# sylvainma/Summarizer

Measured on AMD Instinct MI355X. Metric: frames scored/sec (T x 1024), higher is better.
Workload: dtype f32; 1 GPU; vasnet score, S-TVSum: 50 videos/GPU, T~U(150,320) (sum 12003), D=1024, packed batch; parallelism=video-sharded x1

## Files before the change

summarizer_amd/csrc/attn_b16.hip:

```cpp
#include "pw_common.h"
#include <math.h>
#include <cstdlib>
#include <algorithm>
#include <vector>

namespace sumk {

namespace {

constexpr int AT_ROWS = 64, AT_TMAX = 320, AT_BK = 64;
constexpr int AT_PP = 2 * AT_TMAX + 16;
constexpr int AT_NCH = 256;
constexpr int AT_ROWB = 2 * AT_BK;
constexpr int AT_CROW = 2 * AT_NCH;
constexpr int AT_NST = 3;
constexpr int AT_STAGE1 = (AT_TMAX + AT_ROWS) * AT_ROWB;
constexpr int AT_STAGE2 = AT_BK * AT_CROW;
constexpr int AT_SP = 0;
constexpr int AT_ST2 = 43008;
constexpr int AT_RED = 3 * AT_STAGE1;
constexpr int AT_LDS = AT_RED + 8 * 64 * 4;
static_assert(AT_ROWS * AT_PP <= AT_ST2 && AT_ST2 + 3 * AT_STAGE2 <= AT_RED && AT_LDS <= 160 * 1024, "LDS map");

typedef unsigned int u32x4 __attribute__((ext_vector_type(4)));
typedef float f32x4v __attribute__((ext_vector_type(4)));
typedef __bf16 bf16x4v __attribute__((ext_vector_type(4)));

__device__ __forceinline__ u32x2 pack_bf16x4(float a, float b, float c, float d) {
  return __builtin_bit_cast(u32x2, __builtin_convertvector(f32x4v{a, b, c, d}, bf16x4v));
}


template <bool BWD, int NJ>
__device__ __forceinline__ void attn_strip_body(const AttnStripArgs& a, const SeqInfo& si, const int strip, char* const lds) {
  const int tid = threadIdx.x, lane = tid & 63, li = lane & 31, lh = lane >> 5;
  const int wave = __builtin_amdgcn_readfirstlane(tid >> 6);
  const int T = si.T, i0 = strip * AT_ROWS;
  const Drop drop = drop_resolve(a.drop);
  constexpr int T64 = NJ * 64;
  constexpr int NTW = (2 * NJ + 3) / 4;
  const int D = a.D;
  const int rows = min(AT_ROWS, T - i0);

  const __amdgpu_buffer_rsrc_t rA = __builtin_amdgcn_make_buffer_rsrc(
      const_cast<unsigned short*>(a.A16 + (int64_t)(si.row0 + i0) * a.lda), (short)0, ((rows - 1) * a.lda + D) * 2, 0x00020000);
  const __amdgpu_buffer_rsrc_t rB = __builtin_amdgcn_make_buffer_rsrc(
      const_cast<unsigned short*>(a.B16 + (int64_t)si.row0 * a.ldb), (short)0, ((T - 1) * a.ldb + D) * 2, 0x00020000);
  const int d_row = wave * 8 + (lane >> 3);
  const int d_chunk = (lane & 7) ^ (((lane >> 4) + 4 * (wave & 1)) & 7);
  int vk[NJ];
#pragma unroll
  for (int p = 0; p < NJ; ++p) vk[p] = (min(d_row + 64 * p, T - 1) * a.ldb + d_chunk * 8) * 2;
  const int vq = (min(d_row, rows - 1) * a.lda + d_chunk * 8) * 2;
  constexpr int NI1 = NJ + 1;
  auto dma1 = [&](int kt, int stage) {
    char* const dst = lds + stage * AT_STAGE1 + wave * 1024;
#pragma unroll
    for (int p = 0; p < NJ; ++p)
      __builtin_amdgcn_raw_ptr_buffer_load_lds(rB, (lds_vptr)(dst + p * 8192), 16, vk[p], kt * (AT_BK * 2), 0, 0);
    __builtin_amdgcn_raw_ptr_buffer_load_lds(rA, (lds_vptr)(dst + T64 * AT_ROWB), 16, vq, kt * (AT_BK * 2), 0, 0);
  };
  const int qt = wave & 1, kg = wave >> 1;
  const int sw = (li >> 1) & 7;
  const int fq = (T64 + qt * 32 + li) * AT_ROWB, fk = (kg * 32 + li) * AT_ROWB;
  struct Frag1 { bf16x8 bq, ak[NTW]; };
  auto read1 = [&](const char* buf, int ks, Frag1& f) {
    const int so = ((2 * ks + lh) ^ sw) * 16;
    f.bq = *reinterpret_cast<const bf16x8*>(buf + fq + so);
#pragma unroll
    for (int j = 0; j < NTW; ++j) f.ak[j] = *reinterpret_cast<const bf16x8*>(buf + fk + j * 128 * AT_ROWB + so);
  };
  f32x16 acc[NTW];
#pragma unroll
  for (int j = 0; j < NTW; ++j)
#pragma unroll
    for (int r = 0; r < 16; ++r) acc[j][r] = 0.f;

  const int qi = qt * 32 + li, i = i0 + qi;
  const uint64_t drow = (uint64_t)(si.row0 + i) << 20;
  uint32_t keepm[NTW];
#pragma unroll
  for (int j = 0; j < NTW; ++j) keepm[j] = 0u;
  auto keep_step = [&](int r) {
#pragma unroll
    for (int j = 0; j < NTW; ++j) {
      const int key = (kg + 4 * j) * 32 + 8 * (r >> 2) + 4 * lh + (r & 3);
      keepm[j] |= (dropout_keep(drop.seed, 0, drow | (uint64_t)key, drop.thr) ? 1u : 0u) << r;
    }
  };
  const int KT1 = D / AT_BK;
  dma1(0, 0);
  if (AT_NST > 2) dma1(1, 1);
  int stage = 0;
  for (int kt = 0; kt < KT1; ++kt) {
    if (AT_NST > 2 && kt + 1 < KT1) wait_vm<NI1>(); else wait_vm<0>();
    __builtin_amdgcn_s_barrier();
    const int st2 = stage == 0 ? AT_NST - 1 : stage - 1;
    const char* const cur = lds + stage * AT_STAGE1;
    auto compute1 = [&]() {
      if (drop.thr && kt < 16) keep_step(kt);
      Frag1 f[2];
      read1(cur, 0, f[0]);
#pragma unroll
      for (int ks = 0; ks < AT_BK / 16; ++ks) {
        if (ks + 1 < AT_BK / 16) read1(cur, ks + 1, f[(ks + 1) & 1]);
#pragma unroll
        for (int j = 0; j < NTW; ++j) acc[j] = __builtin_amdgcn_mfma_f32_32x32x16_bf16(f[ks & 1].ak[j], f[ks & 1].bq, acc[j], 0, 0, 0);
      }
    };
    if (wave < 4) {
      if (kt + AT_NST - 1 < KT1) dma1(kt + AT_NST - 1, st2);
      compute1();
    } else {
      compute1();
      if (kt + AT_NST - 1 < KT1) dma1(kt + AT_NST - 1, st2);
    }
    stage = stage == AT_NST - 1 ? 0 : stage + 1;
  }
  if (drop.thr)
    for (int r = KT1; r < 16; ++r) keep_step(r);
  __syncthreads();

  const __amdgpu_buffer_rsrc_t rC = __builtin_amdgcn_make_buffer_rsrc(
      const_cast<unsigned short*>(a.C16 + (int64_t)si.row0 * a.ldc), (short)0, ((T - 1) * a.ldc + D) * 2, 0x00020000);
  const int c_row = wave * 2 + (lane >> 5);
  const int c_chunk = ((((lane & 31) >> 2) ^ (c_row & 3)) << 2) | (lane & 3);
  const int NC = D / AT_NCH, n_it = NC * NJ;
  constexpr int NI2 = 4;
  auto dma2 = [&](int nc, int kt, int stage) {
    char* const dst = lds + AT_ST2 + stage * AT_STAGE2 + wave * 1024;
#pragma unroll
    for (int p = 0; p < 4; ++p)
      __builtin_amdgcn_raw_ptr_buffer_load_lds(rC, (lds_vptr)(dst + p * 8192), 16,
                                               (min(kt * 64 + c_row + 16 * p, T - 1) * a.ldc + nc * AT_NCH + c_chunk * 8) * 2, 0, 0, 0);
  };
  dma2(0, 0, 0);
  if (n_it > 1) dma2(NJ > 1 ? 0 : 1, NJ > 1 ? 1 : 0, 1);

  const bool row_ok = i < T;
  float* const red = reinterpret_cast<float*>(lds + AT_RED);
  float* const erow = a.E + si.eoff + (int64_t)i * si.ldE;
  unsigned short* const prow = a.P16 + si.e16off + (int64_t)i * T64;
  char* const lrow = lds + AT_SP + qi * AT_PP;
  if constexpr (!BWD) {
    float m = -INFINITY;
#pragma unroll
    for (int j = 0; j < NTW; ++j)
#pragma unroll
      for (int r = 0; r < 16; ++r) {
        const int key = (kg + 4 * j) * 32 + 8 * (r >> 2) + 4 * lh + (r & 3);
        const float e = key < T ? masked_logit(acc[j][r], a.scale, i, key, a.ignore_self, a.aperture) : -INFINITY;
        acc[j][r] = e;
        m = fmaxf(m, e);
      }
    m = fmaxf(m, __shfl_xor(m, 32));
    if (lh == 0) red[kg * 64 + qi] = m;
    lds_barrier();
    m = fmaxf(fmaxf(red[qi], red[64 + qi]), fmaxf(red[128 + qi], red[192 + qi]));
    float sum = 0.f;
#pragma unroll
    for (int j = 0; j < NTW; ++j)
#pragma unroll
      for (int r = 0; r < 16; ++r) {
        const int key = (kg + 4 * j) * 32 + 8 * (r >> 2) + 4 * lh + (r & 3);
        const float p = key < T ? __expf(acc[j][r] - m) : 0.f;
        acc[j][r] = p;
        sum += p;
      }
    sum += __shfl_xor(sum, 32);
    if (lh == 0) red[256 + kg * 64 + qi] = sum;
    lds_barrier();
    sum = (red[256 + qi] + red[320 + qi]) + (red[384 + qi] + red[448 + qi]);
    const float rsum = 1.0f / sum;
#pragma unroll
    for (int j = 0; j < NTW; ++j)
#pragma unroll
      for (int g = 0; g < 4; ++g) {
        const int k0 = (kg + 4 * j) * 32 + 8 * g + 4 * lh;
        if (k0 >= T64) continue;
        float al[4], ad[4];
#pragma unroll
        for (int c = 0; c < 4; ++c) {
          al[c] = k0 + c < T ? acc[j][4 * g + c] * rsum : 0.f;
          ad[c] = drop.thr ? (((keepm[j] >> (4 * g + c)) & 1u) ? al[c] * drop.scale : 0.f) : al[c];
        }
        const u32x2 pk = pack_bf16x4(ad[0], ad[1], ad[2], ad[3]);
        if (row_ok) {
          if (k0 < si.ldE) *reinterpret_cast<float4*>(erow + k0) = make_float4(al[0], al[1], al[2], al[3]);
          *reinterpret_cast<u32x2*>(prow + k0) = pk;
        }
        *reinterpret_cast<u32x2*>(lrow + k0 * 2) = row_ok ? pk : u32x2{0u, 0u};
      }
  } else {
    float dot = 0.f;
    float al[NTW][16];
#pragma unroll
    for (int j = 0; j < NTW; ++j)
#pragma unroll
      for (int g = 0; g < 4; ++g) {
        const int k0 = (kg + 4 * j) * 32 + 8 * g + 4 * lh;
        float4 t = make_float4(0.f, 0.f, 0.f, 0.f);
        if (row_ok && k0 < si.ldE) t = *reinterpret_cast<const float4*>(erow + k0);
        al[j][4 * g] = t.x; al[j][4 * g + 1] = t.y; al[j][4 * g + 2] = t.z; al[j][4 * g + 3] = t.w;
      }
#pragma unroll
    for (int j = 0; j < NTW; ++j)
#pragma unroll
      for (int r = 0; r < 16; ++r) {
        float d = acc[j][r];
        if (drop.thr) d = ((keepm[j] >> r) & 1u) ? d * drop.scale : 0.f;
        acc[j][r] = d;
        dot += d * al[j][r];
      }
    dot += __shfl_xor(dot, 32);
    if (lh == 0) red[kg * 64 + qi] = dot;
    lds_barrier();
    dot = (red[qi] + red[64 + qi]) + (red[128 + qi] + red[192 + qi]);
#pragma unroll
    for (int j = 0; j < NTW; ++j)
#pragma unroll
      for (int g = 0; g < 4; ++g) {
        const int k0 = (kg + 4 * j) * 32 + 8 * g + 4 * lh;
        if (k0 >= T64) continue;
        float v[4];
#pragma unroll
        for (int c = 0; c < 4; ++c) v[c] = al[j][4 * g + c] * (acc[j][4 * g + c] - dot) * a.scale;
        const u32x2 pk = row_ok ? pack_bf16x4(v[0], v[1], v[2], v[3]) : u32x2{0u, 0u};
        if (row_ok) *reinterpret_cast<u32x2*>(prow + k0) = pk;
        *reinterpret_cast<u32x2*>(lrow + k0 * 2) = pk;
      }
  }

  const int rr = (lane >> 2) & 3;
  const int fct = (8 * lh + ((lane & 15) >> 2)) * AT_CROW + 32 * ((lane >> 4) & 1) + 8 * (lane & 3) + ((wave ^ rr) << 6);
  const char* const fp = lds + AT_SP + li * AT_PP + 16 * lh;
  struct Frag2 { bf16x8 fa, fb[2]; };
  auto read2 = [&](const char* buf, int kt, int ks, Frag2& f) {
    f.fa = tr_frag(buf + fct + 16 * ks * AT_CROW, AT_CROW);
#pragma unroll
    for (int u = 0; u < 2; ++u) f.fb[u] = *reinterpret_cast<const bf16x8*>(fp + u * 32 * AT_PP + (kt * 64 + ks * 16) * 2);
  };
  int stage2 = 0, it = 0;
  int nc2 = NJ > 2 ? 0 : (NJ == 2 ? 1 : 2), kt2 = NJ > 2 ? 2 : 0;
  for (int nc = 0; nc < NC; ++nc) {
    f32x16 o[2];
#pragma unroll
    for (int u = 0; u < 2; ++u)
#pragma unroll
      for (int r = 0; r < 16; ++r) o[u][r] = 0.f;
#pragma unroll
    for (int kt = 0; kt < NJ; ++kt) {
      if (it + 1 < n_it && !(kt == 0 && nc > 0)) wait_vm<NI2>(); else wait_vm<0>();
      __builtin_amdgcn_s_waitcnt(0xC07F);
      __builtin_amdgcn_s_barrier();
      const int st2 = stage2 == 0 ? 2 : stage2 - 1;
      const char* const cur = lds + AT_ST2 + stage2 * AT_STAGE2;
      auto compute2 = [&]() {
        Frag2 f[2];
        read2(cur, kt, 0, f[0]);
#pragma unroll
        for (int ks = 0; ks < 4; ++ks) {
          if (ks + 1 < 4) read2(cur, kt, ks + 1, f[(ks + 1) & 1]);
#pragma unroll
          for (int u = 0; u < 2; ++u) o[u] = __builtin_amdgcn_mfma_f32_32x32x16_bf16(f[ks & 1].fa, f[ks & 1].fb[u], o[u], 0, 0, 0);
        }
      };
      if (wave < 4) {
        if (it + 2 < n_it) dma2(nc2, kt2, st2);
        compute2();
      } else {
        compute2();
        if (it + 2 < n_it) dma2(nc2, kt2, st2);
      }
      if (++kt2 == NJ) { kt2 = 0; ++nc2; }
      stage2 = stage2 == 2 ? 0 : stage2 + 1;
      ++it;
    }
#pragma unroll
    for (int u = 0; u < 2; ++u) {
      const int q = u * 32 + li;
      unsigned short* const orow = a.O16 + (int64_t)(si.row0 + i0 + q) * a.ldo + nc * AT_NCH + wave * 32 + 4 * lh;
      if (q < rows) {
#pragma unroll
        for (int g = 0; g < 4; ++g)
          *reinterpret_cast<u32x2*>(orow + 8 * g) = pack_bf16x4(o[u][4 * g], o[u][4 * g + 1], o[u][4 * g + 2], o[u][4 * g + 3]);
      }
    }
  }
}

template <bool BWD>
__global__ __launch_bounds__(512) void attn_strip_kernel(AttnStripArgs a) {
  extern __shared__ __attribute__((aligned(16))) char lds[];
  int s, strip;
  SeqInfo si;
  if (!locate_block(a.seq, a.n_seq, [](int t) { return (t + AT_ROWS - 1) / AT_ROWS; }, si, s, strip)) return;
  switch ((si.T + 63) >> 6) {
    case 1: attn_strip_body<BWD, 1>(a, si, strip, lds); break;
    case 2: attn_strip_body<BWD, 2>(a, si, strip, lds); break;
    case 3: attn_strip_body<BWD, 3>(a, si, strip, lds); break;
    case 4: attn_strip_body<BWD, 4>(a, si, strip, lds); break;
    default: attn_strip_body<BWD, 5>(a, si, strip, lds); break;
  }
}

}

bool attn_strip_ok(int t_max, int D, int64_t rows, int ld_max) {
  (void)rows;
  return t_max >= 1 && t_max <= AT_TMAX && D % AT_NCH == 0 && D >= AT_NCH && ((int64_t)(t_max + 64) * ld_max + D) * 2 < ((int64_t)1 << 31);
}

int launch_attn_strip(bool backward, const AttnStripArgs& a_in, hipStream_t stream) {
  const AttnStripArgs& a = a_in;
  SUMK_TRY(backward ? lds_opt_in<attn_strip_kernel<true>>(AT_LDS) : lds_opt_in<attn_strip_kernel<false>>(AT_LDS));
  const unsigned grid = (unsigned)(8 * ((a.n_seq + 7) / 8) * a.strips);
  if (backward) hipLaunchKernelGGL(attn_strip_kernel<true>, dim3(grid), dim3(512), AT_LDS, stream, a);
  else hipLaunchKernelGGL(attn_strip_kernel<false>, dim3(grid), dim3(512), AT_LDS, stream, a);
  SUMK_HIP(hipGetLastError());
  return SUMK_OK;
}

}

static int strips_table(const char* who, int32_t n_seq, const int32_t* seq_off_host, std::vector<sumk::SeqInfo>* h, int64_t* e_elems, int64_t* p16_elems,
                        int* t_max) {
  SUMK_ARG(seq_off_host, "%s: seq_off_host is null", who);
  SUMK_ARG(n_seq >= 1, "%s: n_seq=%d must be at least 1", who, n_seq);
  int64_t eoff = 0, e16off = 0;
  int tm = 0;
  if (h) h->resize(n_seq);
  for (int s = 0; s < n_seq; ++s) {
    const int T = seq_off_host[s + 1] - seq_off_host[s];
    SUMK_ARG(T >= 1 && seq_off_host[s] >= 0, "%s: video %d has %d frames (seq_off_host)", who, s, T);
    if (h) {
      sumk::SeqInfo& q = (*h)[s];
      q.eoff = eoff; q.row0 = seq_off_host[s]; q.T = T; q.ldE = (T + 3) & ~3; q.pad_ = 0; q.e16off = e16off;
    }
    eoff += (int64_t)T * ((T + 3) & ~3); e16off += (int64_t)T * ((T + 63) & ~63); tm = std::max(tm, T);
  }
  if (e_elems) *e_elems = eoff;
  if (p16_elems) *p16_elems = e16off;
  if (t_max) *t_max = tm;
  return SUMK_OK;
}

extern "C" int sumk_attn_strips_b16_sizes(int32_t n_seq, const int32_t* seq_off_host, int64_t* e_elems, int64_t* p16_elems) {
  SUMK_ARG(e_elems && p16_elems, "attn_strips_b16_sizes: e_elems / p16_elems is null");
  *e_elems = 0; *p16_elems = 0;
  return strips_table("attn_strips_b16_sizes", n_seq, seq_off_host, nullptr, e_elems, p16_elems, nullptr);
}

extern "C" int sumk_attn_strips_b16(int32_t backward, const void* A16, int32_t lda, const void* B16, int32_t ldb, const void* C16, int32_t ldc,
                                    void* O16, int32_t ldo, float* E, void* P16, int32_t D, int32_t n_seq, const int32_t* seq_off_host,
                                    float scale, int32_t ignore_self, int32_t aperture, float dropout_p, uint64_t seed, void* stream_) {
  using namespace sumk;
  hipStream_t stream = (hipStream_t)stream_;
  SUMK_ARG(A16, "attn_strips_b16: A16 is null");
  SUMK_ARG(B16, "attn_strips_b16: B16 is null");
  SUMK_ARG(C16, "attn_strips_b16: C16 is null");
  SUMK_ARG(O16, "attn_strips_b16: O16 is null");
  SUMK_ARG(E, "attn_strips_b16: E is null");
  SUMK_ARG(P16, "attn_strips_b16: P16 is null");
  std::vector<SeqInfo> h;
  int t_max = 0;
  SUMK_TRY(strips_table("attn_strips_b16", n_seq, seq_off_host, &h, nullptr, nullptr, &t_max));
  const struct { const char* name; int32_t ld; const void* p; } ops[] = {{"lda", lda, A16}, {"ldb", ldb, B16}, {"ldc", ldc, C16}, {"ldo", ldo, O16}};
  for (const auto& o : ops) {
    SUMK_ARG(o.ld >= D && o.ld % 8 == 0, "attn_strips_b16: %s=%d must be at least D=%d and a multiple of 8", o.name, o.ld, D);
    SUMK_ARG(((uintptr_t)o.p & 15) == 0, "attn_strips_b16: the operand of %s is not 16-byte aligned", o.name);
  }
  SUMK_ARG(((uintptr_t)E & 15) == 0, "attn_strips_b16: E is not 16-byte aligned");
  SUMK_ARG(((uintptr_t)P16 & 15) == 0, "attn_strips_b16: P16 is not 16-byte aligned");
  SUMK_ARG(dropout_p >= 0.f && dropout_p < 1.f, "attn_strips_b16: dropout_p=%g must lie in [0, 1)", (double)dropout_p);
  const int ld_max = std::max(std::max(lda, ldb), std::max(ldc, ldo));
  SUMK_ARG(attn_strip_ok(t_max, D, seq_off_host[n_seq], ld_max), "attn_strips_b16: not eligible (t_max=%d <= 320, D=%d %% 256 == 0, offsets inside 31 bits)",
           t_max, D);
  AttnStripArgs at;
  at.A16 = (const unsigned short*)A16; at.lda = lda; at.B16 = (const unsigned short*)B16; at.ldb = ldb; at.C16 = (const unsigned short*)C16; at.ldc = ldc;
  at.O16 = (unsigned short*)O16; at.ldo = ldo; at.E = E; at.P16 = (unsigned short*)P16;
  at.n_seq = n_seq; at.strips = (t_max + 63) / 64; at.D = D;
  at.scale = scale; at.ignore_self = ignore_self; at.aperture = aperture; at.drop = make_drop(dropout_p, seed);
  SeqInfo* d = nullptr;
  SUMK_HIP(hipMalloc(&d, sizeof(SeqInfo) * n_seq));
  int rc = SUMK_OK;
  const hipError_t e = hipMemcpyAsync(d, h.data(), sizeof(SeqInfo) * n_seq, hipMemcpyHostToDevice, stream);
  if (e != hipSuccess) rc = hip_fail(e, "hipMemcpyAsync(SeqInfo table)");
  at.seq = d;
  if (rc == SUMK_OK) rc = launch_attn_strip(backward != 0, at, stream);
  const hipError_t es = hipStreamSynchronize(stream);
  if (rc == SUMK_OK && es != hipSuccess) rc = hip_fail(es, "hipStreamSynchronize");
  (void)hipFree(d);
  return rc;
}
```

Before: 10.50 million frames/s.

## Split attention strip kernel into producer waves for DMA and consumer waves for MFMA

Adds four dedicated producer waves that issue all buffer-to-LDS loads for both the QK^T stage and the PV stage, while the eight original waves only wait on barriers and run MFMA compute. Each producer covers two consumer waves' load shares, and the barrier counts are matched across the softmax/row phase. The goal is to take load issue and vmcnt waits off the compute waves' critical path. In exchange the block grows to 768 threads, which raises register pressure under the launch bounds, and the barrier-count matching across roles is fragile.

```diff
diff --git a/summarizer_amd/csrc/attn_b16.hip b/summarizer_amd/csrc/attn_b16.hip
--- a/summarizer_amd/csrc/attn_b16.hip
+++ b/summarizer_amd/csrc/attn_b16.hip
@@ -14,6 +14,10 @@
 constexpr int AT_ROWB = 2 * AT_BK;
 constexpr int AT_CROW = 2 * AT_NCH;
 constexpr int AT_NST = 3;
+constexpr int AT_CW = 8, AT_PW = 4;
+constexpr int AT_SH = AT_CW / AT_PW;
+static_assert(AT_PW % 2 == 0 && AT_SH * AT_PW == AT_CW, "a producer's shares are of one parity");
+template <bool BWD> constexpr int AT_ROW_BARRIERS = BWD ? 1 : 2;
 constexpr int AT_STAGE1 = (AT_TMAX + AT_ROWS) * AT_ROWB;
 constexpr int AT_STAGE2 = AT_BK * AT_CROW;
 constexpr int AT_SP = 0;
@@ -30,6 +34,78 @@
   return __builtin_bit_cast(u32x2, __builtin_convertvector(f32x4v{a, b, c, d}, bf16x4v));
 }
 
+
+template <bool BWD, int NJ>
+__device__ __forceinline__ void attn_strip_producer(const AttnStripArgs& a, const SeqInfo& si, const int strip, char* const lds, const int pw) {
+  const int lane = threadIdx.x & 63;
+  const int T = si.T, i0 = strip * AT_ROWS, D = a.D;
+  constexpr int T64 = NJ * 64;
+  const int rows = min(AT_ROWS, T - i0);
+  const __amdgpu_buffer_rsrc_t rA = __builtin_amdgcn_make_buffer_rsrc(
+      const_cast<unsigned short*>(a.A16 + (int64_t)(si.row0 + i0) * a.lda), (short)0, ((rows - 1) * a.lda + D) * 2, 0x00020000);
+  const __amdgpu_buffer_rsrc_t rB = __builtin_amdgcn_make_buffer_rsrc(
+      const_cast<unsigned short*>(a.B16 + (int64_t)si.row0 * a.ldb), (short)0, ((T - 1) * a.ldb + D) * 2, 0x00020000);
+  const int d_chunk = (lane & 7) ^ (((lane >> 4) + 4 * (pw & 1)) & 7);
+  int vk[AT_SH][NJ], vq[AT_SH];
+#pragma unroll
+  for (int h = 0; h < AT_SH; ++h) {
+    const int d_row = (pw + AT_PW * h) * 8 + (lane >> 3);
+#pragma unroll
+    for (int p = 0; p < NJ; ++p) vk[h][p] = (min(d_row + 64 * p, T - 1) * a.ldb + d_chunk * 8) * 2;
+    vq[h] = (min(d_row, rows - 1) * a.lda + d_chunk * 8) * 2;
+  }
+  constexpr int NI1 = AT_SH * (NJ + 1);
+  auto dma1 = [&](int kt, int stage) {
+#pragma unroll
+    for (int h = 0; h < AT_SH; ++h) {
+      char* const dst = lds + stage * AT_STAGE1 + (pw + AT_PW * h) * 1024;
+#pragma unroll
+      for (int p = 0; p < NJ; ++p)
+        __builtin_amdgcn_raw_ptr_buffer_load_lds(rB, (lds_vptr)(dst + p * 8192), 16, vk[h][p], kt * (AT_BK * 2), 0, 0);
+      __builtin_amdgcn_raw_ptr_buffer_load_lds(rA, (lds_vptr)(dst + T64 * AT_ROWB), 16, vq[h], kt * (AT_BK * 2), 0, 0);
+    }
+  };
+  const int KT1 = D / AT_BK;
+  dma1(0, 0);
+  dma1(1, 1);
+  int stage = 0;
+  for (int kt = 0; kt < KT1; ++kt) {
+    if (kt + 1 < KT1) wait_vm<NI1>(); else wait_vm<0>();
+    __builtin_amdgcn_s_barrier();
+    if (kt + AT_NST - 1 < KT1) dma1(kt + AT_NST - 1, stage == 0 ? AT_NST - 1 : stage - 1);
+    stage = stage == AT_NST - 1 ? 0 : stage + 1;
+  }
+  __builtin_amdgcn_s_barrier();
+
+  const __amdgpu_buffer_rsrc_t rC = __builtin_amdgcn_make_buffer_rsrc(
+      const_cast<unsigned short*>(a.C16 + (int64_t)si.row0 * a.ldc), (short)0, ((T - 1) * a.ldc + D) * 2, 0x00020000);
+  const int c_row = pw * 2 + (lane >> 5);
+  const int c_chunk = ((((lane & 31) >> 2) ^ (c_row & 3)) << 2) | (lane & 3);
+  const int NC = D / AT_NCH, n_it = NC * NJ;
+  constexpr int NI2 = 4 * AT_SH;
+  auto dma2 = [&](int nc, int kt, int stage) {
+#pragma unroll
+    for (int h = 0; h < AT_SH; ++h) {
+      char* const dst = lds + AT_ST2 + stage * AT_STAGE2 + (pw + AT_PW * h) * 1024;
+#pragma unroll
+      for (int p = 0; p < 4; ++p)
+        __builtin_amdgcn_raw_ptr_buffer_load_lds(rC, (lds_vptr)(dst + p * 8192), 16,
+                                                 (min(kt * 64 + c_row + 2 * AT_PW * h + 16 * p, T - 1) * a.ldc + nc * AT_NCH + c_chunk * 8) * 2, 0, 0, 0);
+    }
+  };
+  dma2(0, 0, 0);
+  if (n_it > 1) dma2(NJ > 1 ? 0 : 1, NJ > 1 ? 1 : 0, 1);
+  for (int b = 0; b < AT_ROW_BARRIERS<BWD>; ++b) __builtin_amdgcn_s_barrier();
+  int stage2 = 0;
+  int nc2 = NJ > 2 ? 0 : (NJ == 2 ? 1 : 2), kt2 = NJ > 2 ? 2 : 0;
+  for (int it = 0; it < n_it; ++it) {
+    if (it + 1 < n_it) wait_vm<NI2>(); else wait_vm<0>();
+    __builtin_amdgcn_s_barrier();
+    if (it + 2 < n_it) dma2(nc2, kt2, stage2 == 0 ? 2 : stage2 - 1);
+    if (++kt2 == NJ) { kt2 = 0; ++nc2; }
+    stage2 = stage2 == 2 ? 0 : stage2 + 1;
+  }
+}
 
 template <bool BWD, int NJ>
 __device__ __forceinline__ void attn_strip_body(const AttnStripArgs& a, const SeqInfo& si, const int strip, char* const lds) {
@@ -41,25 +117,11 @@
   constexpr int NTW = (2 * NJ + 3) / 4;
   const int D = a.D;
   const int rows = min(AT_ROWS, T - i0);
-
-  const __amdgpu_buffer_rsrc_t rA = __builtin_amdgcn_make_buffer_rsrc(
-      const_cast<unsigned short*>(a.A16 + (int64_t)(si.row0 + i0) * a.lda), (short)0, ((rows - 1) * a.lda + D) * 2, 0x00020000);
-  const __amdgpu_buffer_rsrc_t rB = __builtin_amdgcn_make_buffer_rsrc(
-      const_cast<unsigned short*>(a.B16 + (int64_t)si.row0 * a.ldb), (short)0, ((T - 1) * a.ldb + D) * 2, 0x00020000);
-  const int d_row = wave * 8 + (lane >> 3);
-  const int d_chunk = (lane & 7) ^ (((lane >> 4) + 4 * (wave & 1)) & 7);
-  int vk[NJ];
-#pragma unroll
-  for (int p = 0; p < NJ; ++p) vk[p] = (min(d_row + 64 * p, T - 1) * a.ldb + d_chunk * 8) * 2;
-  const int vq = (min(d_row, rows - 1) * a.lda + d_chunk * 8) * 2;
-  constexpr int NI1 = NJ + 1;
-  auto dma1 = [&](int kt, int stage) {
-    char* const dst = lds + stage * AT_STAGE1 + wave * 1024;
-#pragma unroll
-    for (int p = 0; p < NJ; ++p)
-      __builtin_amdgcn_raw_ptr_buffer_load_lds(rB, (lds_vptr)(dst + p * 8192), 16, vk[p], kt * (AT_BK * 2), 0, 0);
-    __builtin_amdgcn_raw_ptr_buffer_load_lds(rA, (lds_vptr)(dst + T64 * AT_ROWB), 16, vq, kt * (AT_BK * 2), 0, 0);
-  };
+  if (wave >= AT_CW) {
+    attn_strip_producer<BWD, NJ>(a, si, strip, lds, wave - AT_CW);
+    return;
+  }
+
   const int qt = wave & 1, kg = wave >> 1;
   const int sw = (li >> 1) & 7;
   const int fq = (T64 + qt * 32 + li) * AT_ROWB, fk = (kg * 32 + li) * AT_ROWB;
@@ -89,31 +151,18 @@
     }
   };
   const int KT1 = D / AT_BK;
-  dma1(0, 0);
-  if (AT_NST > 2) dma1(1, 1);
   int stage = 0;
   for (int kt = 0; kt < KT1; ++kt) {
-    if (AT_NST > 2 && kt + 1 < KT1) wait_vm<NI1>(); else wait_vm<0>();
     __builtin_amdgcn_s_barrier();
-    const int st2 = stage == 0 ? AT_NST - 1 : stage - 1;
     const char* const cur = lds + stage * AT_STAGE1;
-    auto compute1 = [&]() {
-      if (drop.thr && kt < 16) keep_step(kt);
-      Frag1 f[2];
-      read1(cur, 0, f[0]);
-#pragma unroll
-      for (int ks = 0; ks < AT_BK / 16; ++ks) {
-        if (ks + 1 < AT_BK / 16) read1(cur, ks + 1, f[(ks + 1) & 1]);
-#pragma unroll
-        for (int j = 0; j < NTW; ++j) acc[j] = __builtin_amdgcn_mfma_f32_32x32x16_bf16(f[ks & 1].ak[j], f[ks & 1].bq, acc[j], 0, 0, 0);
-      }
-    };
-    if (wave < 4) {
-      if (kt + AT_NST - 1 < KT1) dma1(kt + AT_NST - 1, st2);
-      compute1();
-    } else {
-      compute1();
-      if (kt + AT_NST - 1 < KT1) dma1(kt + AT_NST - 1, st2);
+    if (drop.thr && kt < 16) keep_step(kt);
+    Frag1 f[2];
+    read1(cur, 0, f[0]);
+#pragma unroll
+    for (int ks = 0; ks < AT_BK / 16; ++ks) {
+      if (ks + 1 < AT_BK / 16) read1(cur, ks + 1, f[(ks + 1) & 1]);
+#pragma unroll
+      for (int j = 0; j < NTW; ++j) acc[j] = __builtin_amdgcn_mfma_f32_32x32x16_bf16(f[ks & 1].ak[j], f[ks & 1].bq, acc[j], 0, 0, 0);
     }
     stage = stage == AT_NST - 1 ? 0 : stage + 1;
   }
@@ -121,21 +170,7 @@
     for (int r = KT1; r < 16; ++r) keep_step(r);
   __syncthreads();
 
-  const __amdgpu_buffer_rsrc_t rC = __builtin_amdgcn_make_buffer_rsrc(
-      const_cast<unsigned short*>(a.C16 + (int64_t)si.row0 * a.ldc), (short)0, ((T - 1) * a.ldc + D) * 2, 0x00020000);
-  const int c_row = wave * 2 + (lane >> 5);
-  const int c_chunk = ((((lane & 31) >> 2) ^ (c_row & 3)) << 2) | (lane & 3);
-  const int NC = D / AT_NCH, n_it = NC * NJ;
-  constexpr int NI2 = 4;
-  auto dma2 = [&](int nc, int kt, int stage) {
-    char* const dst = lds + AT_ST2 + stage * AT_STAGE2 + wave * 1024;
-#pragma unroll
-    for (int p = 0; p < 4; ++p)
-      __builtin_amdgcn_raw_ptr_buffer_load_lds(rC, (lds_vptr)(dst + p * 8192), 16,
-                                               (min(kt * 64 + c_row + 16 * p, T - 1) * a.ldc + nc * AT_NCH + c_chunk * 8) * 2, 0, 0, 0);
-  };
-  dma2(0, 0, 0);
-  if (n_it > 1) dma2(NJ > 1 ? 0 : 1, NJ > 1 ? 1 : 0, 1);
+  const int NC = D / AT_NCH;
 
   const bool row_ok = i < T;
   float* const red = reinterpret_cast<float*>(lds + AT_RED);
@@ -240,8 +275,7 @@
 #pragma unroll
     for (int u = 0; u < 2; ++u) f.fb[u] = *reinterpret_cast<const bf16x8*>(fp + u * 32 * AT_PP + (kt * 64 + ks * 16) * 2);
   };
-  int stage2 = 0, it = 0;
-  int nc2 = NJ > 2 ? 0 : (NJ == 2 ? 1 : 2), kt2 = NJ > 2 ? 2 : 0;
+  int stage2 = 0;
   for (int nc = 0; nc < NC; ++nc) {
     f32x16 o[2];
 #pragma unroll
@@ -250,31 +284,18 @@
       for (int r = 0; r < 16; ++r) o[u][r] = 0.f;
 #pragma unroll
     for (int kt = 0; kt < NJ; ++kt) {
-      if (it + 1 < n_it && !(kt == 0 && nc > 0)) wait_vm<NI2>(); else wait_vm<0>();
       __builtin_amdgcn_s_waitcnt(0xC07F);
       __builtin_amdgcn_s_barrier();
-      const int st2 = stage2 == 0 ? 2 : stage2 - 1;
       const char* const cur = lds + AT_ST2 + stage2 * AT_STAGE2;
-      auto compute2 = [&]() {
-        Frag2 f[2];
-        read2(cur, kt, 0, f[0]);
-#pragma unroll
-        for (int ks = 0; ks < 4; ++ks) {
-          if (ks + 1 < 4) read2(cur, kt, ks + 1, f[(ks + 1) & 1]);
-#pragma unroll
-          for (int u = 0; u < 2; ++u) o[u] = __builtin_amdgcn_mfma_f32_32x32x16_bf16(f[ks & 1].fa, f[ks & 1].fb[u], o[u], 0, 0, 0);
-        }
-      };
-      if (wave < 4) {
-        if (it + 2 < n_it) dma2(nc2, kt2, st2);
-        compute2();
-      } else {
-        compute2();
-        if (it + 2 < n_it) dma2(nc2, kt2, st2);
-      }
-      if (++kt2 == NJ) { kt2 = 0; ++nc2; }
+      Frag2 f[2];
+      read2(cur, kt, 0, f[0]);
+#pragma unroll
+      for (int ks = 0; ks < 4; ++ks) {
+        if (ks + 1 < 4) read2(cur, kt, ks + 1, f[(ks + 1) & 1]);
+#pragma unroll
+        for (int u = 0; u < 2; ++u) o[u] = __builtin_amdgcn_mfma_f32_32x32x16_bf16(f[ks & 1].fa, f[ks & 1].fb[u], o[u], 0, 0, 0);
+      }
       stage2 = stage2 == 2 ? 0 : stage2 + 1;
-      ++it;
     }
 #pragma unroll
     for (int u = 0; u < 2; ++u) {
@@ -290,7 +311,7 @@
 }
 
 template <bool BWD>
-__global__ __launch_bounds__(512) void attn_strip_kernel(AttnStripArgs a) {
+__global__ __launch_bounds__(64 * (AT_CW + AT_PW)) void attn_strip_kernel(AttnStripArgs a) {
   extern __shared__ __attribute__((aligned(16))) char lds[];
   int s, strip;
   SeqInfo si;
@@ -315,8 +336,8 @@
   const AttnStripArgs& a = a_in;
   SUMK_TRY(backward ? lds_opt_in<attn_strip_kernel<true>>(AT_LDS) : lds_opt_in<attn_strip_kernel<false>>(AT_LDS));
   const unsigned grid = (unsigned)(8 * ((a.n_seq + 7) / 8) * a.strips);
-  if (backward) hipLaunchKernelGGL(attn_strip_kernel<true>, dim3(grid), dim3(512), AT_LDS, stream, a);
-  else hipLaunchKernelGGL(attn_strip_kernel<false>, dim3(grid), dim3(512), AT_LDS, stream, a);
+  if (backward) hipLaunchKernelGGL(attn_strip_kernel<true>, dim3(grid), dim3(64 * (AT_CW + AT_PW)), AT_LDS, stream, a);
+  else hipLaunchKernelGGL(attn_strip_kernel<false>, dim3(grid), dim3(64 * (AT_CW + AT_PW)), AT_LDS, stream, a);
   SUMK_HIP(hipGetLastError());
   return SUMK_OK;
 }
```

After: 10.48 million frames/s. No clear change (-0.2%).
